# Epiphany-f/PSL-SLAM

Hardware: AMD Instinct MI355X
Metric: frames/sec ORB+line extract+match, 640x480 RGB-D, 1/2/4/8 MI355X (higher is better)
Workload: dtype u8; 1 GPU; configs[2]: 640x480 synthetic structure scene at the configured line load ('sticks': non-overlapping high-contrast bars), ORB 1000/1.2/8 FAST 20/7 + LSD (LSD_REFINE_ADV) / merge / top-200 / LBD + LIL pairing + RGB-D line glue (isLineGood, crossings, planes) extract, SearchByProjection(cur,last) + LSDmatcher::match, frames resident in HBM; scene=sticks, distinct_frames_per_batch=256, streams=1, launcher=none, multi_gpu=single GPU, lsd_refine=LSD_REFINE_ADV, lbd_sample_bytes_per_frame=2654242

## Files before the change

psl-slam_amd/csrc/line_kernels2.h:

```cpp
#ifndef PSL_LINE_KERNELS2_H
#define PSL_LINE_KERNELS2_H

#include "line_kernels.h"

#define PSL_MERGE_NMAX 4096
#define PSL_MERGE_CLMAX 65536
#define PSL_FAN_CAP PSLFE_FAN_CAP

struct MergeScratch {
    float* lines0;
    float* lines1;
    float* merged;
    float* angles;
    float* length;
    int* order;
    int* pos;
    uint32_t* adj;
    int* code;
    int* clist;
    int* coff;
    int* work;
    uint32_t* bits;
    PslKeyLine* stage;
};

__device__ __forceinline__ float psl_point_line_distance(const float* l, float x0, float y0) {
    const float x1 = l[0], y1 = l[1], x2 = l[2], y2 = l[3];
    const float numf = __builtin_fabsf(PSL_FADD(PSL_FADD(PSL_FMUL(PSL_FSUB(y2, y1), x0), PSL_FMUL(PSL_FSUB(x1, x2), y0)),
                                                PSL_FSUB(PSL_FMUL(x2, y1), PSL_FMUL(x1, y2))));
    const double a = (double)PSL_FSUB(y2, y1), b = (double)PSL_FSUB(x1, x2);
    const double den = __dsqrt_rn(PSL_DADD(PSL_DMUL(a, a), PSL_DMUL(b, b)));
    return (float)((double)numf / den);
}

__device__ __forceinline__ float psl_angle_diff_f(float a1, float a2) {
    const float c1 = __builtin_fabsf(PSL_FSUB(a2, a1));
    const float c2 = (float)PSL_DSUB(PSL_DADD(PSL_PI, (double)fminf(a1, a2)), (double)fmaxf(a1, a2));
    return fminf(c1, c2);
}

__device__ bool psl_merge_pair(const float* src, const float* angles, int idx1, int idx2, float angle_thr, float distance_thr, float ep_thr) {
    float x11 = src[4 * idx1], y11 = src[4 * idx1 + 1], x12 = src[4 * idx1 + 2], y12 = src[4 * idx1 + 3];
    const float angle1 = angles[idx1];
    const bool to_sort_x = __builtin_fabsf(angle1) < (float)(PSL_PI / 4.0);
    if ((to_sort_x && (x12 < x11)) || ((!to_sort_x) && y12 < y11)) { float t = x11; x11 = x12; x12 = t; t = y11; y11 = y12; y12 = t; }
    float x21 = src[4 * idx2], y21 = src[4 * idx2 + 1], x22 = src[4 * idx2 + 2], y22 = src[4 * idx2 + 3];
    if ((to_sort_x && (x22 < x21)) || ((!to_sort_x) && y22 < y21)) { float t = x21; x21 = x22; x22 = t; t = y21; y21 = y22; y22 = t; }
    if (psl_angle_diff_f(angle1, angles[idx2]) > angle_thr) return false;
    const float mid_x1 = (float)PSL_DMUL(0.5, (double)PSL_FADD(src[4 * idx1], src[4 * idx1 + 2]));
    const float mid_y1 = (float)PSL_DMUL(0.5, (double)PSL_FADD(src[4 * idx1 + 1], src[4 * idx1 + 3]));
    const float mid_x2 = (float)PSL_DMUL(0.5, (double)PSL_FADD(src[4 * idx2], src[4 * idx2 + 2]));
    const float mid_y2 = (float)PSL_DMUL(0.5, (double)PSL_FADD(src[4 * idx2 + 1], src[4 * idx2 + 3]));
    const float m1 = psl_point_line_distance(&src[4 * idx2], mid_x1, mid_y1);
    const float m2 = psl_point_line_distance(&src[4 * idx1], mid_x2, mid_y2);
    if (m1 > distance_thr && m2 > distance_thr) return false;
    float cx12, cy12, cx21, cy21;
    if ((to_sort_x && x12 > x22) || (!to_sort_x && y12 > y22)) { cx12 = x22; cy12 = y22; cx21 = x11; cy21 = y11; }
    else { cx12 = x12; cy12 = y12; cx21 = x21; cy21 = y21; }
    bool to_merge = ((to_sort_x && cx12 >= cx21) || (!to_sort_x && cy12 >= cy21));
    if (!to_merge) {
        const float ex = PSL_FSUB(cx21, cx12), ey = PSL_FSUB(cy21, cy12);
        to_merge = PSL_FADD(PSL_FMUL(ex, ex), PSL_FMUL(ey, ey)) < ep_thr;
    }
    return to_merge;
}

__device__ void psl_merge_two_lines(const float* l1, const float* l2, float* out, const double* sctab) {
    const float ax = l1[0], ay = l1[1], bx = l1[2], by = l1[3], cx = l2[0], cy = l2[1], dx = l2[2], dy = l2[3];
    const float dlix = PSL_FSUB(bx, ax), dliy = PSL_FSUB(by, ay), dljx = PSL_FSUB(dx, cx), dljy = PSL_FSUB(dy, cy);
    const double li = __dsqrt_rn(PSL_DADD((double)PSL_FMUL(dlix, dlix), (double)PSL_FMUL(dliy, dliy)));
    const double lj = __dsqrt_rn(PSL_DADD((double)PSL_FMUL(dljx, dljx), (double)PSL_FMUL(dljy, dljy)));
    const double den = PSL_DMUL(2.0, PSL_DADD(li, lj));
    const double xg = PSL_DADD(PSL_DMUL(li, (double)PSL_FADD(ax, bx)), PSL_DMUL(lj, (double)PSL_FADD(cx, dx))) / den;
    const double yg = PSL_DADD(PSL_DMUL(li, (double)PSL_FADD(ay, by)), PSL_DMUL(lj, (double)PSL_FADD(cy, dy))) / den;
    const double thi = dlix == 0.0f ? PSL_PI / 2.0 : (double)psl_atanf(PSL_FDIV(dliy, dlix));
    const double thj = dljx == 0.0f ? PSL_PI / 2.0 : (double)psl_atanf(PSL_FDIV(dljy, dljx));
    double thr;
    if (fabs(PSL_DSUB(thi, thj)) <= PSL_PI / 2.0) thr = PSL_DADD(PSL_DMUL(li, thi), PSL_DMUL(lj, thj)) / PSL_DADD(li, lj);
    else {
        const double tmp = PSL_DSUB(thj, PSL_DMUL(PSL_PI, thj / fabs(thj)));
        thr = PSL_DADD(PSL_DMUL(li, thi), PSL_DMUL(lj, tmp));
        thr = thr / PSL_DADD(li, lj);
    }
    const double s = psl_glibc_sin(thr, sctab), c = psl_glibc_cos(thr, sctab);
    const double axg = PSL_DADD(PSL_DMUL(PSL_DSUB((double)ay, yg), s), PSL_DMUL(PSL_DSUB((double)ax, xg), c));
    const double bxg = PSL_DADD(PSL_DMUL(PSL_DSUB((double)by, yg), s), PSL_DMUL(PSL_DSUB((double)bx, xg), c));
    const double cxg = PSL_DADD(PSL_DMUL(PSL_DSUB((double)cy, yg), s), PSL_DMUL(PSL_DSUB((double)cx, xg), c));
    const double dxg = PSL_DADD(PSL_DMUL(PSL_DSUB((double)dy, yg), s), PSL_DMUL(PSL_DSUB((double)dx, xg), c));
    const double d1 = fmin(axg, fmin(bxg, fmin(cxg, dxg))), d2 = fmax(axg, fmax(bxg, fmax(cxg, dxg)));
    out[0] = (float)PSL_DADD(PSL_DMUL(d1, c), xg); out[1] = (float)PSL_DADD(PSL_DMUL(d1, s), yg);
    out[2] = (float)PSL_DADD(PSL_DMUL(d2, c), xg); out[3] = (float)PSL_DADD(PSL_DMUL(d2, s), yg);
}

#define PSL_MERGE_LDSN 1024
#define PSL_MERGE_LDSN_SMALL 512
__device__ __forceinline__ int psl_block_excl_scan256(int v, int* s_w, int* total);
template <int LN>
struct MergeLds {
    int code[LN], order[LN], pos[LN], tc[LN], nx[LN], loc[LN];
    float length[LN];
    uint32_t bits[LN / 32];
    uint8_t clustered[LN];
    __attribute__((aligned(16))) uint32_t row[PSL_MERGE_NMAX / 32];
};

template <int LN>
__device__ __forceinline__ const uint32_t* psl_merge_row(MergeLds<LN>& LD, const uint32_t* row, int words) {
    const uint4* r4 = reinterpret_cast<const uint4*>(row);
    uint4* d4 = reinterpret_cast<uint4*>(LD.row);
    const int nq = (words + 3) >> 2;
    for (int base = 0; base < nq; base += 8) {
        uint4 t[8];
#pragma unroll
        for (int u = 0; u < 8; ++u) t[u] = base + u < nq ? r4[base + u] : make_uint4(0, 0, 0, 0);
#pragma unroll
        for (int u = 0; u < 8; ++u)
            if (base + u < nq) d4[base + u] = t[u];
    }
    return LD.row;
}

template <int LN>
__device__ int psl_merge_pass(const MergeScratch& M, MergeLds<LN>& LD, const float* src, float* dst, int n, float angle_threshold,
                              float distance_threshold, float endpoint_threshold, float length_thr, int* s_i, const double* sctab) {
    const int tid = threadIdx.x, BS = 256;
    if (n <= 0) return 0;
    const bool small = n <= LN;
    const int words = (n + 31) >> 5;
    const int ROW = PSL_MERGE_NMAX / 32;
    for (int i = tid; i < n; i += BS) {
        const float dx = PSL_FSUB(src[4 * i + 2], src[4 * i]), dy = PSL_FSUB(src[4 * i + 3], src[4 * i + 1]);
        M.angles[i] = psl_atanf(PSL_FDIV(dy, dx));
        const float len = sqrtf(PSL_FADD(PSL_FMUL(dx, dx), PSL_FMUL(dy, dy)));
        M.length[i] = len;
        M.code[i] = -1;
        if (small) { LD.length[i] = len; LD.code[i] = -1; }
    }
    __syncthreads();
    for (int i = tid; i < n; i += BS) {
        const float a = M.angles[i];
        int r = 0;
        for (int j = 0; j < n; ++j) { const float b = M.angles[j]; r += (b < a) || (b == a && j < i); }
        M.pos[i] = r;
        M.order[r] = i;
        if (small) { LD.pos[i] = r; LD.order[r] = i; }
    }
    __syncthreads();
    const float ep_thr = PSL_FMUL(endpoint_threshold, endpoint_threshold);
    if (small) {
        float* sa = reinterpret_cast<float*>(LD.loc);
        int* wm = LD.tc;
        int* pw = LD.nx;
        for (int p = tid; p < n; p += BS) sa[p] = M.angles[LD.order[p]];
        for (int t = tid; t < n * words; t += BS) M.adj[(size_t)(t / words) * ROW + (t % words)] = 0;
        __syncthreads();
        const float tband = angle_threshold + 1e-3f;
        auto lower = [&](float v) { int lo = 0, hi = n; while (lo < hi) { const int mid = (lo + hi) >> 1; if (sa[mid] < v) lo = mid + 1; else hi = mid; } return lo; };
        auto upper = [&](float v) { int lo = 0, hi = n; while (lo < hi) { const int mid = (lo + hi) >> 1; if (sa[mid] <= v) lo = mid + 1; else hi = mid; } return lo; };
        auto span = [](int lo, int hi) -> uint32_t {
            if (lo > hi) return 0u;
            const int a = lo >> 5, b = hi >> 5;
            const uint32_t upto = b >= 31 ? 0xffffffffu : ((1u << (b + 1)) - 1u);
            return upto & ~((1u << a) - 1u);
        };
        __shared__ int s_tot, s_scan[4];
        if (tid == 0) s_tot = 0;
        __syncthreads();
        for (int base = 0; base < n; base += BS) {
            const int pi = base + tid;
            uint32_t m = 0;
            if (pi < n) {
                const float a = sa[pi];
                m = span(lower(a - tband), upper(a + tband) - 1);
                m |= span(lower(a + (float)PSL_PI - tband), n - 1);
                m |= span(0, upper(a - (float)PSL_PI + tband) - 1);
                wm[pi] = (int)m;
            }
            int tot;
            const int ex = psl_block_excl_scan256(__popc(m), s_scan, &tot);
            if (pi < n) pw[pi] = s_tot + ex;
            __syncthreads();
            if (tid == 0) s_tot += tot;
            __syncthreads();
        }
        const int T = s_tot;
        for (int k = tid; k < T; k += BS) {
            int lo = 0, hi = n;
            while (lo < hi) { const int mid = (lo + hi) >> 1; if (pw[mid] <= k) lo = mid + 1; else hi = mid; }
            const int pi = lo - 1;
            uint32_t m = (uint32_t)wm[pi];
            for (int r = k - pw[pi]; r > 0; --r) m &= m - 1;
            const int wj = __ffs(m) - 1;
            uint32_t bw = 0;
            const int idxi = LD.order[pi];
            for (int b = 0; b < 32; ++b) {
                const int pj = wj * 32 + b;
                if (pj >= n || pj == pi) continue;
                const int idxj = LD.order[pj];
                const bool mm = pi < pj ? psl_merge_pair(src, M.angles, idxi, idxj, angle_threshold, distance_threshold, ep_thr)
                                        : psl_merge_pair(src, M.angles, idxj, idxi, angle_threshold, distance_threshold, ep_thr);
                bw |= (uint32_t)mm << b;
            }
            M.adj[(size_t)pi * ROW + wj] = bw;
        }
    } else {
        for (int t = tid; t < n * words; t += BS) {
            const int pi = t / words, wj = t - pi * words;
            uint32_t bw = 0;
            const int idxi = M.order[pi];
            for (int b = 0; b < 32; ++b) {
                const int pj = wj * 32 + b;
                if (pj >= n || pj == pi) continue;
                const int idxj = M.order[pj];
                const bool m = pi < pj ? psl_merge_pair(src, M.angles, idxi, idxj, angle_threshold, distance_threshold, ep_thr)
                                       : psl_merge_pair(src, M.angles, idxj, idxi, angle_threshold, distance_threshold, ep_thr);
                bw |= (uint32_t)m << b;
            }
            M.adj[(size_t)pi * ROW + wj] = bw;
        }
    }
    __syncthreads();
    __shared__ int s_cl[3];
    if (small) {
        if (tid < 64) {
            const int lane = tid;
            const unsigned long long ltm = (1ull << lane) - 1ull;
            int* code = LD.code;
            const int* order = LD.order;
            const int* posv = LD.pos;
            uint32_t* bits = LD.bits;
            int* to_check = LD.tc;
            int* next = LD.nx;
            int* qpos = LD.loc;
            for (int k = lane; k < n; k += 64) qpos[k] = 0x7fffffff;
            if (lane == 0) M.coff[0] = 0;
            __builtin_amdgcn_wave_barrier();
            int ncl = 0, total = 0;
            bool overflow = false;
            for (int i = 0; i < n && !overflow; ++i) {
                if (code[i] >= 0) continue;
                const int new_code = ncl;
                __builtin_amdgcn_wave_barrier();
                if (lane == 0) code[i] = new_code;
                int ntc;
                {
                    uint32_t v = lane < words ? M.adj[(size_t)posv[i] * ROW + lane] : 0u;
                    const int c = __popc(v);
                    int inc = c;
#pragma unroll
                    for (int o = 1; o < 64; o <<= 1) { const int u = __shfl_up(inc, o); if (lane >= o) inc += u; }
                    ntc = __shfl(inc, 63);
                    int o = inc - c;
                    while (v) { const int bb = __ffs(v) - 1; v &= v - 1; to_check[o++] = order[lane * 32 + bb]; }
                }
                if (total < PSL_MERGE_CLMAX) { if (lane == 0) M.clist[total] = i; ++total; } else overflow = true;
                __builtin_amdgcn_wave_barrier();
                while (ntc > 0 && !overflow) {
                    if (lane < words) bits[lane] = 0;
                    for (int q = lane; q < ntc; q += 64) qpos[to_check[q]] = q;
                    __builtin_amdgcn_wave_barrier();
                    for (int base = 0; base < ntc; base += 64) {
                        const int q = base + lane;
                        const int j = q < ntc ? to_check[q] : 0;
                        const bool unc = q < ntc && code[j] < 0;
                        const unsigned long long mu = __ballot(unc);
                        const int at = total + __popcll(mu & ltm);
                        if (unc && at < PSL_MERGE_CLMAX) M.clist[at] = j;
                        total += __popcll(mu);
                        if (total > PSL_MERGE_CLMAX) { total = PSL_MERGE_CLMAX; overflow = true; }
                        if (q < ntc) {
                            const uint32_t* row = M.adj + (size_t)posv[j] * ROW;
                            for (int w = 0; w < words; ++w) {
                                uint32_t v = row[w];
                                while (v) {
                                    const int bb = __ffs(v) - 1; v &= v - 1;
                                    const int k = order[w * 32 + bb];
                                    if (code[k] < 0 && !(qpos[k] <= q)) atomicOr(&bits[k >> 5], 1u << (k & 31));
                                }
                            }
                        }
                    }
                    __builtin_amdgcn_wave_barrier();
                    for (int q = lane; q < ntc; q += 64) {
                        const int j = to_check[q];
                        if (code[j] < 0) code[j] = new_code;
                        qpos[j] = 0x7fffffff;
                    }
                    __builtin_amdgcn_wave_barrier();
                    {
                        uint32_t v = lane < words ? bits[lane] : 0u;
                        const int c = __popc(v);
                        int inc = c;
#pragma unroll
                        for (int o = 1; o < 64; o <<= 1) { const int u = __shfl_up(inc, o); if (lane >= o) inc += u; }
                        ntc = __shfl(inc, 63);
                        int o = inc - c;
                        while (v) { const int bb = __ffs(v) - 1; v &= v - 1; next[o++] = lane * 32 + bb; }
                    }
                    int* t = to_check; to_check = next; next = t;
                    __builtin_amdgcn_wave_barrier();
                }
                ++ncl;
                if (lane == 0) M.coff[ncl] = total;
            }
            if (lane == 0) { s_cl[0] = ncl; s_cl[1] = total; s_cl[2] = overflow ? 1 : 0; }
        }
    } else if (tid == 0) {
        int ncl = 0, total = 0;
        int* code = M.code;
        const int* order = M.order;
        const int* posv = M.pos;
        uint32_t* bits = M.bits;
        int* to_check = M.work;
        int* next = M.work + PSL_MERGE_NMAX;
        bool overflow = false;
        M.coff[0] = 0;
        for (int i = 0; i < n && !overflow; ++i) {
            if (code[i] >= 0) continue;
            const int new_code = ncl;
            code[i] = new_code;
            int ntc = 0;
            {
                const uint32_t* row = psl_merge_row(LD, M.adj + (size_t)posv[i] * ROW, words);
                for (int w = 0; w < words; ++w) { uint32_t v = row[w]; while (v) { const int b = __ffs(v) - 1; v &= v - 1; to_check[ntc++] = order[w * 32 + b]; } }
            }
            if (total < PSL_MERGE_CLMAX) M.clist[total++] = i; else overflow = true;
            while (ntc > 0 && !overflow) {
                for (int w = 0; w < words; ++w) bits[w] = 0;
                for (int q = 0; q < ntc; ++q) {
                    const int j = to_check[q];
                    if (code[j] < 0) { code[j] = new_code; if (total < PSL_MERGE_CLMAX) M.clist[total++] = j; else overflow = true; }
                    const uint32_t* row = psl_merge_row(LD, M.adj + (size_t)posv[j] * ROW, words);
                    for (int w = 0; w < words; ++w) {
                        uint32_t v = row[w];
                        while (v) { const int b = __ffs(v) - 1; v &= v - 1; const int k = order[w * 32 + b]; if (code[k] < 0) bits[k >> 5] |= 1u << (k & 31); }
                    }
                }
                ntc = 0;
                for (int w = 0; w < words; ++w) { uint32_t v = bits[w]; while (v) { const int b = __ffs(v) - 1; v &= v - 1; next[ntc++] = w * 32 + b; } }
                int* t = to_check; to_check = next; next = t;
            }
            M.coff[++ncl] = total;
        }
        s_cl[0] = ncl; s_cl[1] = total; s_cl[2] = overflow ? 1 : 0;
    }
    __syncthreads();
    if (tid == 0) {
        int ncl = s_cl[0], total = s_cl[1];
        bool overflow = s_cl[2] != 0;
        const int* order = small ? LD.order : M.order;
        const int* posv = small ? LD.pos : M.pos;
        const float* length = small ? LD.length : M.length;
        const int raw_ncl = ncl;
        int* loc = small ? LD.loc : M.work + 2 * PSL_MERGE_NMAX;
        uint8_t* clustered = small ? LD.clustered : reinterpret_cast<uint8_t*>(M.work + 3 * PSL_MERGE_NMAX);
        int nfinal = 0;
        int* foff = M.coff + PSL_MERGE_NMAX + 1;
        foff[0] = total;
        for (int c = 0; c < raw_ncl && !overflow; ++c) {
            const int cs = M.coff[c + 1] - M.coff[c];
            int* cl = M.clist + M.coff[c];
            if (cs <= 2) {
                for (int q = 0; q < cs; ++q) { if (total < PSL_MERGE_CLMAX) M.clist[total++] = cl[q]; else overflow = true; }
                foff[++nfinal] = total;
                continue;
            }
            for (int a = 1; a < cs; ++a) {
                const int v = cl[a];
                const float lv = length[v];
                int b = a - 1;
                while (b >= 0 && length[cl[b]] < lv) { cl[b + 1] = cl[b]; --b; }
                cl[b + 1] = v;
            }
            for (int q = 0; q < cs; ++q) { loc[cl[q]] = q; clustered[q] = 0; }
            for (int j = 0; j < cs && !overflow; ++j) {
                if (clustered[j]) continue;
                const int line_idx = cl[j];
                if (total < PSL_MERGE_CLMAX) M.clist[total++] = line_idx; else overflow = true;
                const uint32_t* row = psl_merge_row(LD, M.adj + (size_t)posv[line_idx] * ROW, words);
                for (int w = 0; w < words; ++w) {
                    uint32_t v = row[w];
                    while (v) {
                        const int b = __ffs(v) - 1; v &= v - 1;
                        const int k = order[w * 32 + b];
                        clustered[loc[k]] = 1;
                        if (total < PSL_MERGE_CLMAX) M.clist[total++] = k; else overflow = true;
                    }
                }
                foff[++nfinal] = total;
            }
        }
        s_i[0] = nfinal;
        if (overflow) s_i[1] = 1;
    }
    __syncthreads();
    const int nfinal = s_i[0];
    const int* foff = M.coff + PSL_MERGE_NMAX + 1;
    for (int c = tid; c < nfinal; c += BS) {
        const int* cl = M.clist + foff[c];
        const int cs = foff[c + 1] - foff[c];
        float nl[4] = {src[4 * cl[0]], src[4 * cl[0] + 1], src[4 * cl[0] + 2], src[4 * cl[0] + 3]};
        for (int q = 0; q < cs; ++q) {
            float o[4];
            psl_merge_two_lines(nl, &src[4 * cl[q]], o, sctab);
            nl[0] = o[0]; nl[1] = o[1]; nl[2] = o[2]; nl[3] = o[3];
        }
        M.merged[4 * c] = nl[0]; M.merged[4 * c + 1] = nl[1]; M.merged[4 * c + 2] = nl[2]; M.merged[4 * c + 3] = nl[3];
    }
    __syncthreads();
    if (tid == 0) {
        const float thr2 = PSL_FMUL(length_thr, length_thr);
        int keep = 0;
        for (int c = 0; c < nfinal; ++c) {
            const float* m = M.merged + 4 * c;
            const float dx = PSL_FSUB(m[2], m[0]), dy = PSL_FSUB(m[3], m[1]);
            if (PSL_FADD(PSL_FMUL(dx, dx), PSL_FMUL(dy, dy)) > thr2) {
                dst[4 * keep] = m[0]; dst[4 * keep + 1] = m[1]; dst[4 * keep + 2] = m[2]; dst[4 * keep + 3] = m[3];
                ++keep;
            }
        }
        s_i[0] = keep;
    }
    __syncthreads();
    const int out_n = s_i[0];
    __syncthreads();
    return out_n;
}

__device__ int psl_line_iterator_count(int w, int h, float fx1, float fy1, float fx2, float fy2) {
    long long x1 = psl_cvround_f(fx1), y1 = psl_cvround_f(fy1), x2 = psl_cvround_f(fx2), y2 = psl_cvround_f(fy2);
    if ((unsigned long long)x1 >= (unsigned long long)w || (unsigned long long)x2 >= (unsigned long long)w ||
        (unsigned long long)y1 >= (unsigned long long)h || (unsigned long long)y2 >= (unsigned long long)h) {
        const long long right = w - 1, bottom = h - 1;
        int c1 = (x1 < 0) + (x1 > right) * 2 + (y1 < 0) * 4 + (y1 > bottom) * 8;
        int c2 = (x2 < 0) + (x2 > right) * 2 + (y2 < 0) * 4 + (y2 > bottom) * 8;
        if ((c1 & c2) == 0 && (c1 | c2) != 0) {
            long long a;
            if (c1 & 12) { a = c1 < 8 ? 0 : bottom; x1 += (a - y1) * (x2 - x1) / (y2 - y1); y1 = a; c1 = (x1 < 0) + (x1 > right) * 2; }
            if (c2 & 12) { a = c2 < 8 ? 0 : bottom; x2 += (a - y2) * (x2 - x1) / (y2 - y1); y2 = a; c2 = (x2 < 0) + (x2 > right) * 2; }
            if ((c1 & c2) == 0 && (c1 | c2) != 0) {
                if (c1) { a = c1 == 1 ? 0 : right; y1 += (a - x1) * (y2 - y1) / (x2 - x1); x1 = a; c1 = 0; }
                if (c2) { a = c2 == 1 ? 0 : right; y2 += (a - x2) * (y2 - y1) / (x2 - x1); x2 = a; c2 = 0; }
            }
        }
        if ((c1 | c2) != 0) return 0;
    }
    long long dx = x2 - x1, dy = y2 - y1;
    dx = dx < 0 ? -dx : dx; dy = dy < 0 ? -dy : dy;
    return (int)(dx > dy ? dx : dy) + 1;
}

template <int LN>
__global__ __launch_bounds__(256, LN <= PSL_MERGE_LDSN_SMALL ? 8 : 5) void k_line_merge(LineParams P, MergeScratch M0, const float* __restrict__ seg, const int* __restrict__ nseg,
                                                     PslKeyLine* __restrict__ kls, double* __restrict__ lineEq, int* __restrict__ nkl,
                                                     int* __restrict__ status) {
    __shared__ int s_i[4];
    __shared__ MergeLds<LN> LD;
    const int frame = blockIdx.x, tid = threadIdx.x;
    if ((nseg[frame] <= PSL_MERGE_LDSN_SMALL) != (LN == PSL_MERGE_LDSN_SMALL)) return;
    const size_t f = (size_t)frame;
    MergeScratch M;
    M.lines0 = M0.lines0 + f * PSL_MERGE_NMAX * 4; M.lines1 = M0.lines1 + f * PSL_MERGE_NMAX * 4;
    M.merged = M0.merged + f * PSL_MERGE_NMAX * 4;
    M.angles = M0.angles + f * PSL_MERGE_NMAX; M.length = M0.length + f * PSL_MERGE_NMAX;
    M.order = M0.order + f * PSL_MERGE_NMAX; M.pos = M0.pos + f * PSL_MERGE_NMAX;
    M.adj = M0.adj + f * (size_t)PSL_MERGE_NMAX * (PSL_MERGE_NMAX / 32);
    M.code = M0.code + f * PSL_MERGE_NMAX; M.clist = M0.clist + f * PSL_MERGE_CLMAX;
    M.coff = M0.coff + f * (2 * PSL_MERGE_NMAX + 2); M.work = M0.work + f * 4 * PSL_MERGE_NMAX;
    M.bits = M0.bits + f * (PSL_MERGE_NMAX / 32); M.stage = M0.stage + f * PSL_MERGE_NMAX;
    if (tid == 0) s_i[1] = 0;
    int n = nseg[frame];
    int st = 0;
    if (n > PSL_MERGE_NMAX) { n = PSL_MERGE_NMAX; st |= 1; }
    const float* src = seg + f * P.maxseg * 4;
    for (int i = tid; i < n * 4; i += 256) M.lines0[i] = src[i];
    __syncthreads();
    n = psl_merge_pass(M, LD, M.lines0, M.lines1, n, 0.05f, 5.f, 15.f, 30.f, s_i, P.sctab);
    n = psl_merge_pass(M, LD, M.lines1, M.lines0, n, 0.03f, 3.f, 30.f, 50.f, s_i, P.sctab);
    st |= s_i[1] << 1;
    const float* L = M.lines0;
    PslKeyLine* out = kls + f * P.maxkl;
    float* resp = M.angles;
    for (int i = tid; i < n; i += 256) {
        const float* l = L + 4 * i;
        PslKeyLine kl;
        kl.startPointX = l[0]; kl.startPointY = l[1]; kl.endPointX = l[2]; kl.endPointY = l[3];
        kl.sPointInOctaveX = l[0]; kl.sPointInOctaveY = l[1]; kl.ePointInOctaveX = l[2]; kl.ePointInOctaveY = l[3];
        const double ex = (double)PSL_FSUB(l[0], l[2]), ey = (double)PSL_FSUB(l[1], l[3]);
        kl.lineLength = (float)__dsqrt_rn(PSL_DADD(PSL_DMUL(ex, ex), PSL_DMUL(ey, ey)));
        kl.angle = psl_atan2f(PSL_FSUB(kl.endPointY, kl.startPointY), PSL_FSUB(kl.endPointX, kl.startPointX));
        kl.class_id = i;
        kl.octave = 0;
        kl.size = PSL_FMUL(PSL_FSUB(kl.endPointX, kl.startPointX), PSL_FSUB(kl.endPointY, kl.startPointY));
        kl.pt_x = PSL_FADD(kl.endPointX, kl.startPointX) / 2;
        kl.pt_y = PSL_FADD(kl.endPointY, kl.startPointY) / 2;
        kl.response = PSL_FDIV(kl.lineLength, (float)(P.w > P.h ? P.w : P.h));
        kl.numOfPixels = psl_line_iterator_count(P.w, P.h, l[0], l[1], l[2], l[3]);
        resp[i] = kl.response;
        M.stage[i] = kl;
    }
    __syncthreads();
    int m = n;
    if (n > P.nfeatures) {
        m = P.nfeatures;
        for (int i = tid; i < n; i += 256) {
            const float r = resp[i];
            int rank = 0;
            for (int j = 0; j < n; ++j) { const float q = resp[j]; rank += (q > r) || (q == r && j < i); }
            if (rank < m) { PslKeyLine kl = M.stage[i]; kl.class_id = rank; out[rank] = kl; }
        }
    } else {
        if (m > P.maxkl) { m = P.maxkl; st |= 4; }
        for (int i = tid; i < m; i += 256) out[i] = M.stage[i];
    }
    __syncthreads();
    double* eq = lineEq + f * P.maxkl * 3;
    for (int i = tid; i < m; i += 256) {
        const double sx = out[i].startPointX, sy = out[i].startPointY, ex = out[i].endPointX, ey = out[i].endPointY;
        const double lx = PSL_DSUB(sy, ey), ly = PSL_DSUB(ex, sx), lz = PSL_DSUB(PSL_DMUL(sx, ey), PSL_DMUL(sy, ex));
        const double nrm = __dsqrt_rn(PSL_DADD(PSL_DMUL(lx, lx), PSL_DMUL(ly, ly)));
        eq[3 * i] = lx / nrm; eq[3 * i + 1] = ly / nrm; eq[3 * i + 2] = lz / nrm;
    }
    if (tid == 0) { nkl[frame] = m; status[frame] = st; }
}

__global__ __launch_bounds__(256) void k_lbd_pre(LineParams P, const uint8_t* __restrict__ gray, int stride, size_t fstride,
                                                  short2* __restrict__ dxy, int nframes, int xcd) {
    __shared__ __attribute__((aligned(16))) uint8_t s_in[38 * 72 + 16];
    __shared__ __attribute__((aligned(16))) uint16_t s_row[38 * 68 + 8];
    __shared__ __attribute__((aligned(16))) uint8_t s_bl[34 * 68 + 8];
    const int tid = threadIdx.x;
    int tx, ty, frame;
    if (!psl_tile_frame((P.w + 63) / 64, nframes, xcd, &tx, &ty, &frame)) return;
    const int x0 = tx * 64, y0 = ty * 32;
    const uint8_t* img = gray + (size_t)frame * fstride;
    const bool fast = x0 >= 4 && x0 + 68 <= P.w && ((reinterpret_cast<uintptr_t>(img) | (uintptr_t)stride) & 3) == 0;
    if (fast) {
        for (int k = tid; k < 38 * 18; k += 256) {
            const int r = k / 18, c4 = k - r * 18;
            const int gy = psl_reflect101i(y0 + r - 3, P.h);
            reinterpret_cast<uint32_t*>(s_in)[r * 18 + c4] = *reinterpret_cast<const uint32_t*>(img + (size_t)gy * stride + x0 - 4 + c4 * 4);
        }
    } else {
        for (int k = tid; k < 38 * 72; k += 256) {
            const int r = k / 72, c = k - r * 72;
            s_in[r * 72 + c] = img[(size_t)psl_reflect101i(y0 + r - 3, P.h) * stride + psl_reflect101i(x0 - 4 + c, P.w)];
        }
    }
    __syncthreads();
    typedef unsigned short u16x2 __attribute__((ext_vector_type(2)));
    const uint32_t K0 = (uint32_t)P.lbdK[0], K1 = (uint32_t)P.lbdK[1], K2 = (uint32_t)P.lbdK[2];
    {
        const u16x2 k0 = __builtin_bit_cast(u16x2, K0 * 0x10001u), k1 = __builtin_bit_cast(u16x2, K1 * 0x10001u), k2 = __builtin_bit_cast(u16x2, K2 * 0x10001u);
        for (int k = tid; k < 38 * 17; k += 256) {
            const int r = k / 17, g = k - r * 17;
            const uint32_t* in32 = reinterpret_cast<const uint32_t*>(&s_in[r * 72 + 4 * g]);
            const uint32_t w0 = in32[0], w1 = in32[1], w2 = in32[2];
#define PSL_PAIR(hi, lo, b0, b1) __builtin_bit_cast(u16x2, __builtin_amdgcn_perm(hi, lo, 0x0c000c00u | (uint32_t)(b0) | ((uint32_t)(b1) << 16)))
            const u16x2 p0 = PSL_PAIR(w1, w0, 1, 2), p1 = PSL_PAIR(w1, w0, 2, 3), p2 = PSL_PAIR(w1, w0, 3, 4), p3 = PSL_PAIR(w1, w0, 4, 5);
            const u16x2 p4 = PSL_PAIR(w1, w0, 5, 6), p5 = PSL_PAIR(w1, w0, 6, 7), p6 = PSL_PAIR(w2, w1, 3, 4);
#undef PSL_PAIR
            const u16x2 o01 = k0 * (p0 + p4) + k1 * (p1 + p3) + k2 * p2;
            const u16x2 o23 = k0 * (p2 + p6) + k1 * (p3 + p5) + k2 * p4;
            *reinterpret_cast<uint2*>(&s_row[r * 68 + 4 * g]) = make_uint2(__builtin_bit_cast(uint32_t, o01), __builtin_bit_cast(uint32_t, o23));
        }
    }
    __syncthreads();
    {
        const u16x2 c01 = __builtin_bit_cast(u16x2, K0 | (K1 << 16)), c23 = __builtin_bit_cast(u16x2, K2 | (K1 << 16));
        for (int k = tid; k < 9 * 17; k += 256) {
            const int st = k / 17, g = k - st * 17;
            const int r0 = st * 4;
            uint2 q[8];
#pragma unroll
            for (int rr = 0; rr < 8; ++rr) q[rr] = *reinterpret_cast<const uint2*>(&s_row[min(r0 + rr, 37) * 68 + 4 * g]);
            uint32_t acc[4][4];
#pragma unroll
            for (int i = 0; i < 4; ++i)
#pragma unroll
                for (int x = 0; x < 4; ++x) acc[i][x] = 1u << 15;
#pragma unroll
            for (int rr = 0; rr < 6; ++rr) {
                const u16x2 a0 = __builtin_bit_cast(u16x2, __builtin_amdgcn_perm(q[rr + 1].x, q[rr].x, 0x05040100u));
                const u16x2 a1 = __builtin_bit_cast(u16x2, __builtin_amdgcn_perm(q[rr + 1].x, q[rr].x, 0x07060302u));
                const u16x2 a2 = __builtin_bit_cast(u16x2, __builtin_amdgcn_perm(q[rr + 1].y, q[rr].y, 0x05040100u));
                const u16x2 a3 = __builtin_bit_cast(u16x2, __builtin_amdgcn_perm(q[rr + 1].y, q[rr].y, 0x07060302u));
#pragma unroll
                for (int i = 0; i < 4; ++i) {
                    const int m = rr - i;
                    if (m == 0 || m == 2) {
                        const u16x2 c = m == 0 ? c01 : c23;
                        acc[i][0] = __builtin_amdgcn_udot2(a0, c, acc[i][0], false);
                        acc[i][1] = __builtin_amdgcn_udot2(a1, c, acc[i][1], false);
                        acc[i][2] = __builtin_amdgcn_udot2(a2, c, acc[i][2], false);
                        acc[i][3] = __builtin_amdgcn_udot2(a3, c, acc[i][3], false);
                    }
                }
            }
#pragma unroll
            for (int i = 0; i < 4; ++i) {
                if (r0 + i >= 34) break;
                const uint2 t = q[i + 4];
                acc[i][0] += K0 * (t.x & 0xffff); acc[i][1] += K0 * (t.x >> 16);
                acc[i][2] += K0 * (t.y & 0xffff); acc[i][3] += K0 * (t.y >> 16);
                const uint32_t m0 = min(acc[i][0], 0xffffffu), m1 = min(acc[i][1], 0xffffffu);
                const uint32_t m2 = min(acc[i][2], 0xffffffu), m3 = min(acc[i][3], 0xffffffu);
                const uint32_t lo = __builtin_amdgcn_perm(m1, m0, 0x0c0c0602u), hi = __builtin_amdgcn_perm(m3, m2, 0x06020c0cu);
                *reinterpret_cast<uint32_t*>(&s_bl[(r0 + i) * 68 + 4 * g]) = lo | hi;
            }
        }
    }
    __syncthreads();
    for (int k = tid; k < 32 * 16; k += 256) {
        const int oy = k >> 4, g = k & 15;
        const int x = x0 + 4 * g, y = y0 + oy;
        if (x >= P.w || y >= P.h) continue;
        int c[3][6];
#pragma unroll
        for (int rr = 0; rr < 3; ++rr) {
            const uint32_t* b32 = reinterpret_cast<const uint32_t*>(&s_bl[(oy + rr) * 68 + 4 * g]);
            const uint32_t w0 = b32[0], w1 = b32[1];
            c[rr][0] = w0 & 255; c[rr][1] = (w0 >> 8) & 255; c[rr][2] = (w0 >> 16) & 255; c[rr][3] = w0 >> 24;
            c[rr][4] = w1 & 255; c[rr][5] = (w1 >> 8) & 255;
        }
        short2 o[4];
#pragma unroll
        for (int j = 0; j < 4; ++j) {
            const int a00 = c[0][j], a01 = c[0][j + 1], a02 = c[0][j + 2], a10 = c[1][j], a12 = c[1][j + 2], a20 = c[2][j], a21 = c[2][j + 1], a22 = c[2][j + 2];
            o[j] = make_short2((short)((a02 + 2 * a12 + a22) - (a00 + 2 * a10 + a20)), (short)((a20 + 2 * a21 + a22) - (a00 + 2 * a01 + a02)));
        }
        short2* dst = dxy + (size_t)frame * P.w * P.h + (size_t)y * P.w + x;
        if ((P.w & 3) == 0 && x + 3 < P.w) {
            *reinterpret_cast<uint4*>(dst) = make_uint4(__builtin_bit_cast(uint32_t, o[0]), __builtin_bit_cast(uint32_t, o[1]),
                                                        __builtin_bit_cast(uint32_t, o[2]), __builtin_bit_cast(uint32_t, o[3]));
        } else {
// ... 291 lines not shown
```

Measured before the change: 32700 frames/s.

## Keep line-merge pass fully in LDS with compact adjacency and parallel cluster split

```diff
diff --git a/psl-slam_amd/csrc/line_kernels2.h b/psl-slam_amd/csrc/line_kernels2.h
--- a/psl-slam_amd/csrc/line_kernels2.h
+++ b/psl-slam_amd/csrc/line_kernels2.h
@@ -97,11 +97,25 @@
 __device__ __forceinline__ int psl_block_excl_scan256(int v, int* s_w, int* total);
 template <int LN>
 struct MergeLds {
-    int code[LN], order[LN], pos[LN], tc[LN], nx[LN], loc[LN];
+    static constexpr int ADJCAP = 2048;
+    static constexpr int CLCAP = 2048;
+    __attribute__((aligned(16))) float lines[4 * LN];
+    float angles[LN];
     float length[LN];
+    uint32_t adjc[ADJCAP];
+    uint32_t wm[LN];
+    int coff[LN + 1], foff[LN + 1];
+    uint16_t clist[CLCAP];
+    uint16_t pw[LN];
+    int16_t code[LN];
+    uint16_t order[LN], pos[LN], nx[LN];
+    union {
+        float sa[LN];
+        struct { uint16_t loc[LN], tc[LN]; };
+    };
     uint32_t bits[LN / 32];
     uint8_t clustered[LN];
-    __attribute__((aligned(16))) uint32_t row[PSL_MERGE_NMAX / 32];
+    __attribute__((aligned(16))) uint32_t row[LN > PSL_MERGE_LDSN_SMALL ? PSL_MERGE_NMAX / 32 : 4];
 };
 
 template <int LN>
@@ -120,39 +134,48 @@
     return LD.row;
 }
 
+template <class F>
+__device__ __forceinline__ void psl_merge_row_each(const uint32_t* r, uint32_t m, bool compact, F f) {
+    int c = 0;
+    while (m) {
+        const int w = __ffs(m) - 1;
+        m &= m - 1;
+        uint32_t v = r[compact ? c : w];
+        ++c;
+        while (v) { const int b = __ffs(v) - 1; v &= v - 1; f(w * 32 + b); }
+    }
+}
+
 template <int LN>
-__device__ int psl_merge_pass(const MergeScratch& M, MergeLds<LN>& LD, const float* src, float* dst, int n, float angle_threshold,
-                              float distance_threshold, float endpoint_threshold, float length_thr, int* s_i, const double* sctab) {
+__device__ int psl_merge_pass_lds(const MergeScratch& M, MergeLds<LN>& LD, int n, float angle_threshold, float distance_threshold,
+                                  float endpoint_threshold, float length_thr, int* s_i, const double* sctab) {
     const int tid = threadIdx.x, BS = 256;
+    constexpr int K = LN / 256;
     if (n <= 0) return 0;
-    const bool small = n <= LN;
     const int words = (n + 31) >> 5;
     const int ROW = PSL_MERGE_NMAX / 32;
+    const float* src = LD.lines;
     for (int i = tid; i < n; i += BS) {
         const float dx = PSL_FSUB(src[4 * i + 2], src[4 * i]), dy = PSL_FSUB(src[4 * i + 3], src[4 * i + 1]);
-        M.angles[i] = psl_atanf(PSL_FDIV(dy, dx));
-        const float len = sqrtf(PSL_FADD(PSL_FMUL(dx, dx), PSL_FMUL(dy, dy)));
-        M.length[i] = len;
-        M.code[i] = -1;
-        if (small) { LD.length[i] = len; LD.code[i] = -1; }
+        LD.angles[i] = psl_atanf(PSL_FDIV(dy, dx));
+        LD.length[i] = sqrtf(PSL_FADD(PSL_FMUL(dx, dx), PSL_FMUL(dy, dy)));
+        LD.code[i] = -1;
     }
     __syncthreads();
     for (int i = tid; i < n; i += BS) {
-        const float a = M.angles[i];
+        const float a = LD.angles[i];
         int r = 0;
-        for (int j = 0; j < n; ++j) { const float b = M.angles[j]; r += (b < a) || (b == a && j < i); }
-        M.pos[i] = r;
-        M.order[r] = i;
-        if (small) { LD.pos[i] = r; LD.order[r] = i; }
+        for (int j = 0; j < n; ++j) { const float b = LD.angles[j]; r += (b < a) || (b == a && j < i); }
+        LD.pos[i] = (uint16_t)r;
+        LD.order[r] = (uint16_t)i;
     }
     __syncthreads();
     const float ep_thr = PSL_FMUL(endpoint_threshold, endpoint_threshold);
-    if (small) {
-        float* sa = reinterpret_cast<float*>(LD.loc);
-        int* wm = LD.tc;
-        int* pw = LD.nx;
-        for (int p = tid; p < n; p += BS) sa[p] = M.angles[LD.order[p]];
-        for (int t = tid; t < n * words; t += BS) M.adj[(size_t)(t / words) * ROW + (t % words)] = 0;
+    __shared__ int s_tot, s_scan[4];
+    {
+        const float* sa = LD.sa;
+        for (int p = tid; p < n; p += BS) LD.sa[p] = LD.angles[LD.order[p]];
+        if (tid == 0) s_tot = 0;
         __syncthreads();
         const float tband = angle_threshold + 1e-3f;
         auto lower = [&](float v) { int lo = 0, hi = n; while (lo < hi) { const int mid = (lo + hi) >> 1; if (sa[mid] < v) lo = mid + 1; else hi = mid; } return lo; };
@@ -163,9 +186,6 @@
             const uint32_t upto = b >= 31 ? 0xffffffffu : ((1u << (b + 1)) - 1u);
             return upto & ~((1u << a) - 1u);
         };
-        __shared__ int s_tot, s_scan[4];
-        if (tid == 0) s_tot = 0;
-        __syncthreads();
         for (int base = 0; base < n; base += BS) {
             const int pi = base + tid;
             uint32_t m = 0;
@@ -174,21 +194,25 @@
                 m = span(lower(a - tband), upper(a + tband) - 1);
                 m |= span(lower(a + (float)PSL_PI - tband), n - 1);
                 m |= span(0, upper(a - (float)PSL_PI + tband) - 1);
-                wm[pi] = (int)m;
+                LD.wm[pi] = m;
             }
             int tot;
             const int ex = psl_block_excl_scan256(__popc(m), s_scan, &tot);
-            if (pi < n) pw[pi] = s_tot + ex;
+            if (pi < n) LD.pw[pi] = (uint16_t)(s_tot + ex);
             __syncthreads();
             if (tid == 0) s_tot += tot;
             __syncthreads();
         }
-        const int T = s_tot;
+    }
+    const int T = s_tot;
+    const bool adj_lds = T <= MergeLds<LN>::ADJCAP;
+    {
+        const uint16_t* pw = LD.pw;
         for (int k = tid; k < T; k += BS) {
             int lo = 0, hi = n;
             while (lo < hi) { const int mid = (lo + hi) >> 1; if (pw[mid] <= k) lo = mid + 1; else hi = mid; }
             const int pi = lo - 1;
-            uint32_t m = (uint32_t)wm[pi];
+            uint32_t m = LD.wm[pi];
             for (int r = k - pw[pi]; r > 0; --r) m &= m - 1;
             const int wj = __ffs(m) - 1;
             uint32_t bw = 0;
@@ -197,119 +221,257 @@
                 const int pj = wj * 32 + b;
                 if (pj >= n || pj == pi) continue;
                 const int idxj = LD.order[pj];
-                const bool mm = pi < pj ? psl_merge_pair(src, M.angles, idxi, idxj, angle_threshold, distance_threshold, ep_thr)
-                                        : psl_merge_pair(src, M.angles, idxj, idxi, angle_threshold, distance_threshold, ep_thr);
+                const bool mm = pi < pj ? psl_merge_pair(src, LD.angles, idxi, idxj, angle_threshold, distance_threshold, ep_thr)
+                                        : psl_merge_pair(src, LD.angles, idxj, idxi, angle_threshold, distance_threshold, ep_thr);
                 bw |= (uint32_t)mm << b;
             }
-            M.adj[(size_t)pi * ROW + wj] = bw;
-        }
-    } else {
-        for (int t = tid; t < n * words; t += BS) {
-            const int pi = t / words, wj = t - pi * words;
-            uint32_t bw = 0;
-            const int idxi = M.order[pi];
-            for (int b = 0; b < 32; ++b) {
-                const int pj = wj * 32 + b;
-                if (pj >= n || pj == pi) continue;
-                const int idxj = M.order[pj];
-                const bool m = pi < pj ? psl_merge_pair(src, M.angles, idxi, idxj, angle_threshold, distance_threshold, ep_thr)
-                                       : psl_merge_pair(src, M.angles, idxj, idxi, angle_threshold, distance_threshold, ep_thr);
-                bw |= (uint32_t)m << b;
-            }
-            M.adj[(size_t)pi * ROW + wj] = bw;
-        }
-    }
-    __syncthreads();
-    __shared__ int s_cl[3];
-    if (small) {
-        if (tid < 64) {
-            const int lane = tid;
-            const unsigned long long ltm = (1ull << lane) - 1ull;
-            int* code = LD.code;
-            const int* order = LD.order;
-            const int* posv = LD.pos;
-            uint32_t* bits = LD.bits;
-            int* to_check = LD.tc;
-            int* next = LD.nx;
-            int* qpos = LD.loc;
-            for (int k = lane; k < n; k += 64) qpos[k] = 0x7fffffff;
-            if (lane == 0) M.coff[0] = 0;
+            if (adj_lds) LD.adjc[k] = bw; else M.adj[(size_t)pi * ROW + wj] = bw;
+        }
+    }
+    __syncthreads();
+    auto row_of = [&](int p) -> const uint32_t* { return adj_lds ? LD.adjc + LD.pw[p] : M.adj + (size_t)p * ROW; };
+    __shared__ int s_cl[2];
+    if (tid < 64) {
+        const int lane = tid;
+        const unsigned long long ltm = (1ull << lane) - 1ull;
+        int16_t* code = LD.code;
+        const uint16_t* order = LD.order;
+        const uint16_t* posv = LD.pos;
+        uint32_t* bits = LD.bits;
+        uint16_t* to_check = LD.tc;
+        uint16_t* next = LD.nx;
+        uint16_t* qpos = LD.loc;
+        uint16_t* clist = LD.clist;
+        for (int k = lane; k < n; k += 64) qpos[k] = 0xffff;
+        if (lane == 0) LD.coff[0] = 0;
+        __builtin_amdgcn_wave_barrier();
+        int ncl = 0, total = 0;
+        for (int i = 0; i < n; ++i) {
+            if (code[i] >= 0) continue;
+            const int new_code = ncl;
             __builtin_amdgcn_wave_barrier();
-            int ncl = 0, total = 0;
-            bool overflow = false;
-            for (int i = 0; i < n && !overflow; ++i) {
-                if (code[i] >= 0) continue;
-                const int new_code = ncl;
+            if (lane == 0) code[i] = (int16_t)new_code;
+            int ntc;
+            {
+                const int p = posv[i];
+                const uint32_t m = LD.wm[p];
+                uint32_t v = 0;
+                if (lane < words && ((m >> lane) & 1u)) v = adj_lds ? LD.adjc[LD.pw[p] + __popc(m & ((1u << lane) - 1u))] : M.adj[(size_t)p * ROW + lane];
+                const int c = __popc(v);
+                int inc = c;
+#pragma unroll
+                for (int o = 1; o < 64; o <<= 1) { const int u = __shfl_up(inc, o); if (lane >= o) inc += u; }
+                ntc = __shfl(inc, 63);
+                int o = inc - c;
+                while (v) { const int bb = __ffs(v) - 1; v &= v - 1; to_check[o++] = order[lane * 32 + bb]; }
+            }
+            if (lane == 0 && total < n) clist[total] = (uint16_t)i;
+            ++total;
+            __builtin_amdgcn_wave_barrier();
+            while (ntc > 0) {
+                if (lane < words) bits[lane] = 0;
+                for (int q = lane; q < ntc; q += 64) qpos[to_check[q]] = (uint16_t)q;
                 __builtin_amdgcn_wave_barrier();
-                if (lane == 0) code[i] = new_code;
-                int ntc;
+                for (int base = 0; base < ntc; base += 64) {
+                    const int q = base + lane;
+                    const int j = q < ntc ? to_check[q] : 0;
+                    const bool unc = q < ntc && code[j] < 0;
+                    const unsigned long long mu = __ballot(unc);
+                    const int at = total + __popcll(mu & ltm);
+                    if (unc && at < n) clist[at] = (uint16_t)j;
+                    total += __popcll(mu);
+                    if (q < ntc) {
+                        const int p = posv[j];
+                        psl_merge_row_each(row_of(p), LD.wm[p], adj_lds, [&](int pk) {
+                            const int k = order[pk];
+                            if (code[k] < 0 && !(qpos[k] <= q)) atomicOr(&bits[k >> 5], 1u << (k & 31));
+                        });
+                    }
+                }
+                __builtin_amdgcn_wave_barrier();
+                for (int q = lane; q < ntc; q += 64) {
+                    const int j = to_check[q];
+                    if (code[j] < 0) code[j] = (int16_t)new_code;
+                    qpos[j] = 0xffff;
+                }
+                __builtin_amdgcn_wave_barrier();
                 {
-                    uint32_t v = lane < words ? M.adj[(size_t)posv[i] * ROW + lane] : 0u;
+                    uint32_t v = lane < words ? bits[lane] : 0u;
                     const int c = __popc(v);
                     int inc = c;
 #pragma unroll
                     for (int o = 1; o < 64; o <<= 1) { const int u = __shfl_up(inc, o); if (lane >= o) inc += u; }
                     ntc = __shfl(inc, 63);
                     int o = inc - c;
-                    while (v) { const int bb = __ffs(v) - 1; v &= v - 1; to_check[o++] = order[lane * 32 + bb]; }
+                    while (v) { const int bb = __ffs(v) - 1; v &= v - 1; next[o++] = (uint16_t)(lane * 32 + bb); }
                 }
-                if (total < PSL_MERGE_CLMAX) { if (lane == 0) M.clist[total] = i; ++total; } else overflow = true;
+                uint16_t* t = to_check; to_check = next; next = t;
                 __builtin_amdgcn_wave_barrier();
-                while (ntc > 0 && !overflow) {
-                    if (lane < words) bits[lane] = 0;
-                    for (int q = lane; q < ntc; q += 64) qpos[to_check[q]] = q;
-                    __builtin_amdgcn_wave_barrier();
-                    for (int base = 0; base < ntc; base += 64) {
-                        const int q = base + lane;
-                        const int j = q < ntc ? to_check[q] : 0;
-                        const bool unc = q < ntc && code[j] < 0;
-                        const unsigned long long mu = __ballot(unc);
-                        const int at = total + __popcll(mu & ltm);
-                        if (unc && at < PSL_MERGE_CLMAX) M.clist[at] = j;
-                        total += __popcll(mu);
-                        if (total > PSL_MERGE_CLMAX) { total = PSL_MERGE_CLMAX; overflow = true; }
-                        if (q < ntc) {
-                            const uint32_t* row = M.adj + (size_t)posv[j] * ROW;
-                            for (int w = 0; w < words; ++w) {
-                                uint32_t v = row[w];
-                                while (v) {
-                                    const int bb = __ffs(v) - 1; v &= v - 1;
-                                    const int k = order[w * 32 + bb];
-                                    if (code[k] < 0 && !(qpos[k] <= q)) atomicOr(&bits[k >> 5], 1u << (k & 31));
-                                }
-                            }
-                        }
-                    }
-                    __builtin_amdgcn_wave_barrier();
-                    for (int q = lane; q < ntc; q += 64) {
-                        const int j = to_check[q];
-                        if (code[j] < 0) code[j] = new_code;
-                        qpos[j] = 0x7fffffff;
-                    }
-                    __builtin_amdgcn_wave_barrier();
-                    {
-                        uint32_t v = lane < words ? bits[lane] : 0u;
-                        const int c = __popc(v);
-                        int inc = c;
-#pragma unroll
-                        for (int o = 1; o < 64; o <<= 1) { const int u = __shfl_up(inc, o); if (lane >= o) inc += u; }
-                        ntc = __shfl(inc, 63);
-                        int o = inc - c;
-                        while (v) { const int bb = __ffs(v) - 1; v &= v - 1; next[o++] = lane * 32 + bb; }
-                    }
-                    int* t = to_check; to_check = next; next = t;
-                    __builtin_amdgcn_wave_barrier();
+            }
+            ++ncl;
+            if (lane == 0) LD.coff[ncl] = total < n ? total : n;
+        }
+        if (lane == 0) { s_cl[0] = ncl; s_cl[1] = 0; }
+    }
+    __syncthreads();
+    const int ncl = s_cl[0];
+    int nlist[K], nent[K], lbase[K], ebase[K];
+#pragma unroll
+    for (int u = 0; u < K; ++u) {
+        const int c = u * BS + tid;
+        nlist[u] = 0; nent[u] = 0;
+        if (c < ncl) {
+            const int b0 = LD.coff[c], cs = LD.coff[c + 1] - b0;
+            uint16_t* cl = LD.clist + b0;
+            if (cs <= 2) { nlist[u] = 1; nent[u] = cs; }
+            else {
+                for (int a = 1; a < cs; ++a) {
+                    const uint16_t v = cl[a];
+                    const float lv = LD.length[v];
+                    int b = a - 1;
+                    while (b >= 0 && LD.length[cl[b]] < lv) { cl[b + 1] = cl[b]; --b; }
+                    cl[b + 1] = v;
                 }
-                ++ncl;
-                if (lane == 0) M.coff[ncl] = total;
-            }
-            if (lane == 0) { s_cl[0] = ncl; s_cl[1] = total; s_cl[2] = overflow ? 1 : 0; }
-        }
-    } else if (tid == 0) {
+                uint8_t* clustered = LD.clustered + b0;
+                for (int q = 0; q < cs; ++q) { LD.loc[cl[q]] = (uint16_t)q; clustered[q] = 0; }
+                int nl = 0, ne = 0;
+                for (int j = 0; j < cs; ++j) {
+                    if (clustered[j]) continue;
+                    ++nl; ++ne;
+                    const int p = LD.pos[cl[j]];
+                    psl_merge_row_each(row_of(p), LD.wm[p], adj_lds, [&](int pk) { clustered[LD.loc[LD.order[pk]]] = 1; ++ne; });
+                }
+                nlist[u] = nl; nent[u] = ne;
+            }
+        }
+    }
+    int nfinal = 0, total = n;
+#pragma unroll
+    for (int u = 0; u < K; ++u) {
+        int t;
+        lbase[u] = nfinal + psl_block_excl_scan256(nlist[u], s_scan, &t);
+        nfinal += t;
+        ebase[u] = total + psl_block_excl_scan256(nent[u], s_scan, &t);
+        total += t;
+    }
+    const bool cl_lds = total <= MergeLds<LN>::CLCAP;
+    const bool overflow = total > PSL_MERGE_CLMAX;
+    uint16_t* fl = cl_lds ? LD.clist : reinterpret_cast<uint16_t*>(M.clist);
+    const int flcap = cl_lds ? MergeLds<LN>::CLCAP : PSL_MERGE_CLMAX;
+#pragma unroll
+    for (int u = 0; u < K; ++u) {
+        const int c = u * BS + tid;
+        if (c < ncl) {
+            const int b0 = LD.coff[c], cs = LD.coff[c + 1] - b0;
+            const uint16_t* cl = LD.clist + b0;
+            int li = lbase[u], at = ebase[u];
+            auto open = [&]() { if (at <= PSL_MERGE_CLMAX) { LD.foff[li] = at; if (overflow) atomicMax(&s_cl[1], li + 1); } ++li; };
+            auto put = [&](int v) { if (at < flcap) fl[at] = (uint16_t)v; ++at; };
+            if (cs <= 2) {
+                open();
+                for (int q = 0; q < cs; ++q) put(cl[q]);
+            } else {
+                const uint8_t* clustered = LD.clustered + b0;
+                for (int j = 0; j < cs; ++j) {
+                    if (clustered[j]) continue;
+                    open();
+                    put(cl[j]);
+                    const int p = LD.pos[cl[j]];
+                    psl_merge_row_each(row_of(p), LD.wm[p], adj_lds, [&](int pk) { put(LD.order[pk]); });
+                }
+            }
+        }
+    }
+    __syncthreads();
+    if (overflow) nfinal = s_cl[1];
+    if (tid == 0) {
+        LD.foff[nfinal] = overflow ? PSL_MERGE_CLMAX : total;
+        if (overflow) s_i[1] = 1;
+    }
+    __syncthreads();
+    const float thr2 = PSL_FMUL(length_thr, length_thr);
+    float ml[K][4];
+    bool keep[K];
+#pragma unroll
+    for (int u = 0; u < K; ++u) {
+        const int c = u * BS + tid;
+        keep[u] = false;
+        ml[u][0] = ml[u][1] = ml[u][2] = ml[u][3] = 0.f;
+        if (c < nfinal) {
+            const int b0 = LD.foff[c], cs = LD.foff[c + 1] - b0;
+            if (cs > 0) {
+                const uint16_t* cl = fl + b0;
+                const int first = cl[0];
+                float nl[4] = {src[4 * first], src[4 * first + 1], src[4 * first + 2], src[4 * first + 3]};
+                for (int q = 0; q < cs; ++q) {
+                    float o[4];
+                    psl_merge_two_lines(nl, &src[4 * cl[q]], o, sctab);
+                    nl[0] = o[0]; nl[1] = o[1]; nl[2] = o[2]; nl[3] = o[3];
+                }
+                const float dx = PSL_FSUB(nl[2], nl[0]), dy = PSL_FSUB(nl[3], nl[1]);
+                keep[u] = PSL_FADD(PSL_FMUL(dx, dx), PSL_FMUL(dy, dy)) > thr2;
+                ml[u][0] = nl[0]; ml[u][1] = nl[1]; ml[u][2] = nl[2]; ml[u][3] = nl[3];
+            }
+        }
+    }
+    __syncthreads();
+    int out_n = 0;
+#pragma unroll
+    for (int u = 0; u < K; ++u) {
+        int t;
+        const int at = out_n + psl_block_excl_scan256(keep[u] ? 1 : 0, s_scan, &t);
+        if (keep[u]) { float* d = LD.lines + 4 * at; d[0] = ml[u][0]; d[1] = ml[u][1]; d[2] = ml[u][2]; d[3] = ml[u][3]; }
+        out_n += t;
+    }
+    __syncthreads();
+    return out_n;
+}
+
+template <int LN>
+__device__ int psl_merge_pass_hbm(const MergeScratch& M, MergeLds<LN>& LD, const float* src, float* dst, int n, float angle_threshold,
+                                  float distance_threshold, float endpoint_threshold, float length_thr, int* s_i, const double* sctab) {
+    const int tid = threadIdx.x, BS = 256;
+    if (n <= 0) return 0;
+    const int words = (n + 31) >> 5;
+    const int ROW = PSL_MERGE_NMAX / 32;
+    for (int i = tid; i < n; i += BS) {
+        const float dx = PSL_FSUB(src[4 * i + 2], src[4 * i]), dy = PSL_FSUB(src[4 * i + 3], src[4 * i + 1]);
+        M.angles[i] = psl_atanf(PSL_FDIV(dy, dx));
+        M.length[i] = sqrtf(PSL_FADD(PSL_FMUL(dx, dx), PSL_FMUL(dy, dy)));
+        M.code[i] = -1;
+    }
+    __syncthreads();
+    for (int i = tid; i < n; i += BS) {
+        const float a = M.angles[i];
+        int r = 0;
+        for (int j = 0; j < n; ++j) { const float b = M.angles[j]; r += (b < a) || (b == a && j < i); }
+        M.pos[i] = r;
+        M.order[r] = i;
+    }
+    __syncthreads();
+    const float ep_thr = PSL_FMUL(endpoint_threshold, endpoint_threshold);
+    for (int t = tid; t < n * words; t += BS) {
+        const int pi = t / words, wj = t - pi * words;
+        uint32_t bw = 0;
+        const int idxi = M.order[pi];
+        for (int b = 0; b < 32; ++b) {
+            const int pj = wj * 32 + b;
+            if (pj >= n || pj == pi) continue;
+            const int idxj = M.order[pj];
+            const bool m = pi < pj ? psl_merge_pair(src, M.angles, idxi, idxj, angle_threshold, distance_threshold, ep_thr)
+                                   : psl_merge_pair(src, M.angles, idxj, idxi, angle_threshold, distance_threshold, ep_thr);
+            bw |= (uint32_t)m << b;
+        }
+        M.adj[(size_t)pi * ROW + wj] = bw;
+    }
+    __syncthreads();
+    int* foff = M.coff + PSL_MERGE_NMAX + 1;
+    if (tid == 0) {
         int ncl = 0, total = 0;
         int* code = M.code;
         const int* order = M.order;
         const int* posv = M.pos;
+        const float* length = M.length;
         uint32_t* bits = M.bits;
         int* to_check = M.work;
         int* next = M.work + PSL_MERGE_NMAX;
@@ -342,20 +504,10 @@
             }
             M.coff[++ncl] = total;
         }
-        s_cl[0] = ncl; s_cl[1] = total; s_cl[2] = overflow ? 1 : 0;
-    }
-    __syncthreads();
-    if (tid == 0) {
-        int ncl = s_cl[0], total = s_cl[1];
-        bool overflow = s_cl[2] != 0;
-        const int* order = small ? LD.order : M.order;
-        const int* posv = small ? LD.pos : M.pos;
-        const float* length = small ? LD.length : M.length;
         const int raw_ncl = ncl;
-        int* loc = small ? LD.loc : M.work + 2 * PSL_MERGE_NMAX;
-        uint8_t* clustered = small ? LD.clustered : reinterpret_cast<uint8_t*>(M.work + 3 * PSL_MERGE_NMAX);
+        int* loc = M.work + 2 * PSL_MERGE_NMAX;
+        uint8_t* clustered = reinterpret_cast<uint8_t*>(M.work + 3 * PSL_MERGE_NMAX);
         int nfinal = 0;
-        int* foff = M.coff + PSL_MERGE_NMAX + 1;
         foff[0] = total;
         for (int c = 0; c < raw_ncl && !overflow; ++c) {
             const int cs = M.coff[c + 1] - M.coff[c];
@@ -395,7 +547,6 @@
     }
     __syncthreads();
     const int nfinal = s_i[0];
-    const int* foff = M.coff + PSL_MERGE_NMAX + 1;
     for (int c = tid; c < nfinal; c += BS) {
         const int* cl = M.clist + foff[c];
         const int cs = foff[c + 1] - foff[c];
@@ -451,7 +602,7 @@
 }
 
 template <int LN>
-__global__ __launch_bounds__(256, LN <= PSL_MERGE_LDSN_SMALL ? 8 : 5) void k_line_merge(LineParams P, MergeScratch M0, const float* __restrict__ seg, const int* __restrict__ nseg,
+__global__ __launch_bounds__(256, LN <= PSL_MERGE_LDSN_SMALL ? 4 : 2) void k_line_merge(LineParams P, MergeScratch M0, const float* __restrict__ seg, const int* __restrict__ nseg,
                                                      PslKeyLine* __restrict__ kls, double* __restrict__ lineEq, int* __restrict__ nkl,
                                                      int* __restrict__ status) {
     __shared__ int s_i[4];
@@ -473,14 +624,28 @@
     int st = 0;
     if (n > PSL_MERGE_NMAX) { n = PSL_MERGE_NMAX; st |= 1; }
     const float* src = seg + f * P.maxseg * 4;
-    for (int i = tid; i < n * 4; i += 256) M.lines0[i] = src[i];
-    __syncthreads();
-    n = psl_merge_pass(M, LD, M.lines0, M.lines1, n, 0.05f, 5.f, 15.f, 30.f, s_i, P.sctab);
-    n = psl_merge_pass(M, LD, M.lines1, M.lines0, n, 0.03f, 3.f, 30.f, 50.f, s_i, P.sctab);
+    bool lds = n <= LN;
+    if (lds) { for (int i = tid; i < n * 4; i += 256) LD.lines[i] = src[i]; }
+    else { for (int i = tid; i < n * 4; i += 256) M.lines0[i] = src[i]; }
+    __syncthreads();
+    if (lds) {
+        n = psl_merge_pass_lds(M, LD, n, 0.05f, 5.f, 15.f, 30.f, s_i, P.sctab);
+        n = psl_merge_pass_lds(M, LD, n, 0.03f, 3.f, 30.f, 50.f, s_i, P.sctab);
+    } else if constexpr (LN > PSL_MERGE_LDSN_SMALL) {
+        n = psl_merge_pass_hbm(M, LD, M.lines0, M.lines1, n, 0.05f, 5.f, 15.f, 30.f, s_i, P.sctab);
+        lds = n <= LN;
+        if (lds) {
+            for (int i = tid; i < n * 4; i += 256) LD.lines[i] = M.lines1[i];
+            __syncthreads();
+            n = psl_merge_pass_lds(M, LD, n, 0.03f, 3.f, 30.f, 50.f, s_i, P.sctab);
+        } else {
+            n = psl_merge_pass_hbm(M, LD, M.lines1, M.lines0, n, 0.03f, 3.f, 30.f, 50.f, s_i, P.sctab);
+        }
+    }
     st |= s_i[1] << 1;
-    const float* L = M.lines0;
+    const float* L = lds ? LD.lines : M.lines0;
+    float* resp = lds ? LD.angles : M.angles;
     PslKeyLine* out = kls + f * P.maxkl;
-    float* resp = M.angles;
     for (int i = tid; i < n; i += 256) {
         const float* l = L + 4 * i;
         PslKeyLine kl;
```

New measurement: 33050 frames/s, median of 6. +1.1%, better.
